# liangxuy/ReGenNet

Hardware: AMD Instinct MI355X
Metric: sampled motions/sec (higher is better)
Workload: dtype bf16 MFMA operands, fp32 accumulate/LayerNorm/softmax, for 990 of 1000 steps; fp16 MFMA operands for the next 8; split-bf16 (x3) for the last 2; 1 GPU; ntu: [B=256/GPU,56,6,60] online/concat/no_cond L8 d512, 1000-step DDPM, Philox noise, hipGraph=on; batch_per_gpu=256, global_batch=256, denoiser_evals_per_motion=1000, parallelism=batch-shard x1

## Files before the change

regennet_amd/csrc/rgn_layers.hip:

```cpp
#include "rgn_internal.h"
#include "rgn_device.h"
#include "rgn_tail.h"
#include "rgn_sampler.h"

#include <hip/hip_runtime.h>

#include <cmath>
#include <type_traits>
#include <utility>

namespace rgn {

#ifndef RGN_LY_ST_AUX
#define RGN_LY_ST_AUX 16
#endif

constexpr int LY_NTH = 512, LY_KB = 4096;
constexpr int LY_X = 0, LY_Y = 64 * 1024, LY_EXCH = LY_Y, LY_RED = 128 * 1024, LY_REDF = 2 * 8 * 64, LY_VEC = LY_RED + 2 * LY_REDF * 4, LY_VECW = 640,
              LY_LDS = 160 * 1024;
constexpr int LY_PF = LY_VEC + 8 * LY_VECW * 4;
static_assert(LY_PF + 8 * 256 <= LY_LDS, "LDS map");
enum { V_BO = 0, V_G1 = 64, V_G2 = 128, V_B2 = 192, V_SPV = 256, V_BF1 = 320 , V_BF2 = 448, V_G3 = 512, V_B3 = 576 };
constexpr int LY_RDA = 6;
constexpr int LY_RDM = 8;
struct LYT {
    static constexpr int MT = 2, NT = 2, NW = 8, R = 64, RD = LY_RDM, KB = LY_KB, RED = LY_RED, REDF = LY_REDF;
};

#ifdef RGN_LY_STAMPS
__device__ long long g_ly_st[1024][16];
#define RGN_LYT(i)                                                                                   \
    {                                                                                                \
        __builtin_amdgcn_sched_barrier(0);                                                           \
        if (threadIdx.x == 0 && blockIdx.x < 1024 && l == RGN_LY_STAMPS) g_ly_st[blockIdx.x][i] = __builtin_readcyclecounter(); \
        __builtin_amdgcn_sched_barrier(0);                                                           \
    }
#define RGN_LYS(i)                                                                                   \
    {                                                                                                \
        __builtin_amdgcn_sched_barrier(0);                                                           \
        if (threadIdx.x == 0 && blockIdx.x < 1024 && it == 1) g_ly_st[blockIdx.x][i] = __builtin_readcyclecounter(); \
        __builtin_amdgcn_sched_barrier(0);                                                           \
    }
#else
#define RGN_LYT(i)
#define RGN_LYS(i)
#endif

constexpr int LY_XLD = 356, LY_TILE = 0, LY_XIMG = 92160, LY_NKX = 11;
static_assert(64 * LY_XLD * 4 <= LY_XIMG && LY_XIMG + LY_NKX * 4096 <= LY_LDS, "step boundary LDS map");

template <bool STEPS, bool GUIDED = false, bool F16 = false, bool INPAINT = false>
__global__ __launch_bounds__(LY_NTH, 2) void k_layers(LayersArgs g) {
    static_assert(STEPS || !GUIDED, "guidance inside the launch needs the step boundary");
    static_assert(STEPS || !INPAINT, "in-painting (rgn_set_inpainting) belongs to the step boundary");
    using OP = OpFmt<F16>;
    using op_t = typename OP::t;
    using op8 = typename OP::v8;
    using op4 = typename OP::v4;
    extern __shared__ __attribute__((aligned(16))) char smem[];
    const int tid = threadIdx.x, lane = tid & 63;
    const int wave = __builtin_amdgcn_readfirstlane(tid >> 6);
    const int wn = wave & 3, hg = wave >> 2;
    const int l31 = lane & 31, kh = lane >> 5;
    const int b = xcd_affine(blockIdx.x, gridDim.x), Tq = g.Tq;
    const size_t row0 = (size_t)b * Tq;
#ifdef RGN_LY_PRIO
    if (wave >= 4) __builtin_amdgcn_s_setprio(RGN_LY_PRIO);
#endif
    float* vec = reinterpret_cast<float*>(smem + LY_VEC) + wave * LY_VECW;
    const int lane16 = lane * 16;
    tile_dma_in(smem + LY_X, g.h, g.rows, row0, Tq, lane, wave);
    const int first_step = (g.stepvec || STEPS) ? *g.d_step : 0;
    const TailLane tl = tail_lane<LYT>(smem, lane, wave);
    static_assert(LY_X == 0, "a_off addresses the image at byte 0");
    int a_off[2], a_offy[2];
    tail_a_off(a_off, lane);
    tail_a_off(a_offy, a_off, LY_Y);
    using Pass = TailPass;
    op8 wf[LY_RDM][2];
    const float qs2 = g.qscale * 1.44269504088896340736f;

    f32x4 qb[4];
    float vb1;
    auto load_qbias = [&](const float* bqkv, int r) {
        const float* bq = bqkv + (2 * r + hg) * 128 + wn * 32;
#pragma unroll
        for (int i4 = 0; i4 < 4; ++i4) qb[i4] = *reinterpret_cast<const f32x4*>(bq + 8 * i4 + 4 * kh);
        vb1 = bq[1024 + l31];
    };

    wait_vmcnt<0>();
    __builtin_amdgcn_s_barrier();
    load_qbias(g.lw[0].bqkv, 0);

    const int nit = STEPS ? g.steps : 1;
    auto out_proj = [&](f32x16 (&acc)[2][2], int wv) {
#pragma unroll
        for (int a2 = 0; a2 < 2; ++a2)
#pragma unroll
            for (int b2 = 0; b2 < 2; ++b2)
#pragma unroll
                for (int i = 0; i < 16; ++i) acc[a2][b2][i] = 0.f;
        if (wv < 6) {
            const int cb0 = 2 * wv;
            const Pass p_out{__builtin_amdgcn_make_buffer_rsrc(const_cast<__bf16*>(g.Wout) + (size_t)cb0 * 1024, 0, (16 * g.nb_out - cb0) * 2048, 0x00020000), LY_NKX * 2048, 0};
#pragma unroll
            for (int s2 = 0; s2 < LY_RDM - 1; ++s2) tail_load_g<OP, LYT>(wf, tl, p_out, s2, s2);
            tail_gemm<OP, LYT, 32, false, 0>(acc, wf, tl, a_off, p_out, p_out);
        }
    };
    for (int it = 0; it < nit; ++it) {
    const int step = first_step - it;
    for (int pass = 0; pass < (GUIDED ? 2 : 1); ++pass) {
    if (GUIDED && pass == 1) {
        f32x16 accp[2][2];
        int wave_p = wave, lane_p = lane, b_p = b;
        asm volatile("" : "+s"(wave_p), "+s"(b_p));
        asm volatile("" : "+v"(lane_p));
        out_proj(accp, wave_p);
        if (wave_p < 6) {
            float* pk = g.park + ((size_t)b_p * 6 + wave_p) * 4096 + lane_p * 4;
#pragma unroll
            for (int nt = 0; nt < 2; ++nt)
#pragma unroll
                for (int mt = 0; mt < 2; ++mt)
#pragma unroll
                    for (int i4 = 0; i4 < 4; ++i4)
                        *reinterpret_cast<f32x4*>(pk + ((nt * 2 + mt) * 4 + i4) * 256) = f32x4{accp[nt][mt][4 * i4], accp[nt][mt][4 * i4 + 1], accp[nt][mt][4 * i4 + 2], accp[nt][mt][4 * i4 + 3]};
        }
        __builtin_amdgcn_s_barrier();
        tile_dma_in<16>(smem + LY_X, g.h, g.rows, g.half + (size_t)b_p * Tq, Tq, lane_p, wave_p);
        wait_vmcnt<0>();
        __builtin_amdgcn_s_barrier();
    }
    for (int l = 0; l < g.L; ++l) {
        const LayerWts& w = g.lw[l];
        RGN_LYT(0)
        op4 attk[2][2][4];
        float bo_r = 0.f;
        {
            struct PassA { __amdgpu_buffer_rsrc_t rs; };
            auto qrs = [&](int r) {
                const int blk = (2 * r + hg) * 4 + wn;
                return __builtin_amdgcn_make_buffer_rsrc(const_cast<__bf16*>(w.Wqkv) + (size_t)blk * 1024, 0, 3 * 512 * 512 * 2 - blk * 2048, 0x00020000);
            };
            const PassA pa[2] = {{qrs(0)}, {qrs(1)}};
            op8 wq[LY_RDA][3];
            auto load_ga = [&](const PassA& ps, int hs, int slot) {
                int soff;
                asm volatile("s_mov_b32 %0, %1" : "=s"(soff) : "i"(frag_granule(hs, 48 * 2048)));
#pragma unroll
                for (int t = 0; t < 3; ++t)
                    wq[slot][t] = __builtin_bit_cast(op8, __builtin_amdgcn_raw_buffer_load_b128(ps.rs, lane16, soff + t * (16 * 2048), 0));
            };
            constexpr int AH = LY_RDA - 1;
#pragma unroll
            for (int s = 0; s < AH; ++s) load_ga(pa[0], s, s);
#pragma unroll
            for (int r = 0; r < 2; ++r) {
                const int head = 2 * r + hg;
                f32x16 acc[2][3];
#pragma unroll
                for (int ta = 0; ta < 2; ++ta)
#pragma unroll
                    for (int i4 = 0; i4 < 4; ++i4)
#pragma unroll
                        for (int e = 0; e < 4; ++e) {
                            acc[ta][0][4 * i4 + e] = qb[i4][e];
                            acc[ta][1][4 * i4 + e] = 0.f;
                            acc[ta][2][4 * i4 + e] = vb1;
                        }
                __builtin_amdgcn_sched_barrier(0);
                {
                    op8 af[2];
#pragma unroll
                    for (int ta = 0; ta < 2; ++ta) af[ta] = *reinterpret_cast<const op8*>(smem + a_off[0] + ta * 2048);
#pragma unroll
                    for (int hs = 0; hs < 32; ++hs) {
                        op8 afn[2];
#pragma unroll
                        for (int ta = 0; ta < 2; ++ta) {
                            afn[ta] = af[ta];
                            if (hs + 1 < 32) afn[ta] = *reinterpret_cast<const op8*>(smem + ((hs + 1) >> 1) * LY_KB + a_off[(hs + 1) & 1] + ta * 2048);
                        }
                        if (hs + AH < 32) load_ga(pa[r], hs + AH, (32 * r + hs + AH) % LY_RDA);
                        else if (r == 0) load_ga(pa[1], hs + AH - 32, (32 * r + hs + AH) % LY_RDA);
                        if (hs + AH < 32 || r == 0) {
                            if (hs < AH) wait_vmcnt<3 * AH + 5>();
                            else wait_vmcnt<3 * AH>();
                        }
                        const int slot = (32 * r + hs) % LY_RDA;
#pragma unroll
                        for (int t = 0; t < 3; ++t)
#pragma unroll
                            for (int ta = 0; ta < 2; ++ta) {
                                if (t < 2) acc[ta][t] = OP::mfma(wq[slot][t], af[ta], acc[ta][t]);
                                else acc[ta][t] = OP::mfma(af[ta], wq[slot][t], acc[ta][t]);
                            }
#pragma unroll
                        for (int ta = 0; ta < 2; ++ta) af[ta] = afn[ta];
                    }
                }
// ... 120 lines not shown
                RGN_LYT(3 + 3 * r)
            }
        }
        const Pass p_wo{tail_wrs(w.Wo, 2 * wave, 512 * 512 * 2), 16 * 2048, 0}, p_w1a{tail_wrs(w.W1, 2 * wave, 1024 * 512 * 2), 32 * 2048, 0},
            p_w1b{tail_wrs(w.W1, 16 + 2 * wave, 1024 * 512 * 2), 32 * 2048, 0}, p_w2a{tail_wrs(w.W2, 2 * wave, 512 * 1024 * 2), 16 * 2048, 0},
            p_w2b{p_w2a.rs, 16 * 2048, 32};
        vec[V_BO + lane] = bo_r;
#pragma unroll
        for (int s = 0; s < LY_RDM - 1; ++s) tail_load_g<OP, LYT>(wf, tl, p_wo, s, s);
        int cw = 64 * wave + lane;
        asm volatile("" : "+v"(cw));
        float vv[12];
        {
            const float* src[9] = {w.bo, w.g1, w.g2, w.b2, w.bf1, w.bf1 + 512, w.bf2, w.g3, w.b3};
            vv[1] = src[1][cw]; vv[2] = src[2][cw]; vv[3] = src[3][cw];
            vv[4] = w.b1[cw] + (g.stepvec ? g.stepvec[(size_t)step * g.ldstep + (size_t)l * 512 + cw] : 0.f) +
                    (g.pervec ? g.pervec[((size_t)b + (size_t)pass * g.B) * g.ldper + (size_t)l * 512 + cw] : 0.f);
            vv[5] = src[4][cw]; vv[6] = src[5][cw]; vv[7] = src[6][cw]; vv[8] = src[7][cw]; vv[9] = src[8][cw];
        }
        asm volatile("" ::: "memory");
#pragma unroll
        for (int r = 0; r < 2; ++r)
#pragma unroll
            for (int qtile = 0; qtile < 2; ++qtile)
#pragma unroll
                for (int i4 = 0; i4 < 4; ++i4)
                    *reinterpret_cast<op4*>(smem + LY_Y + ((2 * r + hg) * 4 + wn) * LY_KB + (32 * qtile + l31) * 64 + img_slot(i4, tl.swz) + 8 * kh) = attk[r][qtile][i4];
        wait_lgkmcnt<0>();
        __builtin_amdgcn_s_barrier();
        f32x16 acc[2][2];
        tail_init_bias<LYT>(acc, tl, vec + V_BO);
        RGN_LYT(7)
        tail_gemm<OP, LYT, 32, true, 11>(acc, wf, tl, a_offy, p_wo, p_w1a);
        RGN_LYT(8)
        vec[V_G1 + lane] = vv[1]; vec[V_G2 + lane] = vv[2]; vec[V_B2 + lane] = vv[3]; vec[V_SPV + lane] = vv[4];
        vec[V_BF1 + lane] = vv[5]; vec[V_BF1 + 64 + lane] = vv[6]; vec[V_BF2 + lane] = vv[7]; vec[V_G3 + lane] = vv[8]; vec[V_B3 + lane] = vv[9];
        tail_add_resid<OP, LYT>(acc, tl, LY_X);
        tail_layernorm<LYT, 0>(acc, tl, vec + V_G1, tail_rowvec(tl, vec + V_SPV));
        tail_layernorm<LYT, 1>(acc, tl, vec + V_G2, tail_rowvec(tl, vec + V_B2));
        tail_store_img<OP, LYT>(acc, tl, LY_X);
        wait_lgkmcnt<0>();
        __builtin_amdgcn_s_barrier();
        RGN_LYT(9)
        f32x16 acc2[2][2];
        tail_ffn<OP, LYT>(acc2, wf, tl, a_off, a_offy, LY_Y, p_w1a, p_w1b, p_w2a, p_w2b, vec + V_BF1, vec + V_BF2);
        load_qbias(g.lw[l + 1 < g.L ? l + 1 : 0].bqkv, 0);
#ifndef RGN_LY_NO_PREFETCH
        if constexpr (STEPS) {
            if (l == g.L - 1) {
                const int nsl = (int)(gridDim.x >> 3) >= 32 ? 32 : ((int)(gridDim.x >> 3) > 0 ? (int)(gridDim.x >> 3) : 1);
                const int sl = (int)(blockIdx.x >> 3) % nsl;
                const int n_out = 16 * g.nb_out * 16, n_all = n_out + LY_NKX * 16 * 16;
                const unsigned pf_lds = (unsigned)(size_t)((RGN_AS3 char*)(smem + LY_PF)) + (unsigned)wave * 256u;
                for (int ln = sl + nsl * tid; ln < n_all; ln += nsl * LY_NTH) {
                    const char* pp = ln < n_out ? reinterpret_cast<const char*>(g.Wout) + (size_t)ln * 128 : reinterpret_cast<const char*>(g.Wx) + (size_t)(ln - n_out) * 128;
                    int m0_keep;
                    asm volatile("s_mov_b32 %0, m0\n\ts_mov_b32 m0, %2\n\ts_nop 0\n\tglobal_load_lds_dword %1, off\n\ts_mov_b32 m0, %0" : "=&s"(m0_keep) : "v"(pp), "s"(pf_lds) : "memory");
                }
            }
        }
#endif
        RGN_LYT(10)
        tail_add_resid<OP, LYT>(acc2, tl, LY_X);
        tail_layernorm<LYT, 0>(acc2, tl, vec + V_G3, tail_rowvec(tl, vec + V_B3));
        tail_store_img<OP, LYT>(acc2, tl, LY_X);
        wait_lgkmcnt<0>();
        __builtin_amdgcn_s_barrier();
        RGN_LYT(11)
    }
    }
    if constexpr (STEPS) {
        int lane_s = lane, wave_s = wave, b_s = b;
        asm volatile("" : "+v"(lane_s));
        asm volatile("" : "+s"(wave_s), "+s"(b_s));
        const int l31_s = lane_s & 31, kh_s = lane_s >> 5;
        const size_t row0_s = (size_t)b_s * Tq;
        auto col4s = [&](int nt, int i4) { return 32 * nt + 8 * i4 + 4 * kh_s; };
        RGN_LYS(12)
        const SampleParams sp = *g.sp;
        const StepCoef k = g.tab[step];
        const int T = Tq, gb = g.s0 + b_s;
        const float gscale = GUIDED ? g.scale[gb] : 0.f;
        const __amdgpu_buffer_rsrc_t park_rs = __builtin_amdgcn_make_buffer_rsrc(GUIDED ? g.park + ((size_t)b_s * 6 + (wave_s < 6 ? wave_s : 0)) * 4096 : nullptr, 0, 4096 * 4, 0x00020000);
        f32x16 acc[2][2];
        out_proj(acc, wave_s);
        __builtin_amdgcn_s_barrier();
        float* tile = reinterpret_cast<float*>(smem + LY_TILE);
#pragma unroll
        for (int nt = 0; nt < 2; ++nt)
#pragma unroll
            for (int i4 = 0; i4 < 4; ++i4) {
                const int n = 64 * wave_s + col4s(nt, i4);
                if (n < 352) {
                    f32x4 bb = {0.f, 0.f, 0.f, 0.f};
                    if (n < g.F) bb = *reinterpret_cast<const f32x4*>(g.bout + n);
#pragma unroll
                    for (int mt = 0; mt < 2; ++mt) {
                        f32x4 v = {acc[nt][mt][4 * i4] + bb[0], acc[nt][mt][4 * i4 + 1] + bb[1], acc[nt][mt][4 * i4 + 2] + bb[2], acc[nt][mt][4 * i4 + 3] + bb[3]};
                        if constexpr (GUIDED) {
                            const f32x4 cc = __builtin_bit_cast(f32x4, __builtin_amdgcn_raw_buffer_load_b128(park_rs, (lane_s * 4 + ((nt * 2 + mt) * 4 + i4) * 256) * 4, 0, 16));
#pragma unroll
                            for (int e = 0; e < 4; ++e) v[e] = guide(cc[e] + bb[e], v[e], gscale);
                        }
                        *reinterpret_cast<f32x4*>(tile + (32 * mt + l31_s) * LY_XLD + n) = v;
                    }
                }
            }
        const Pass p_wx{__builtin_amdgcn_make_buffer_rsrc(const_cast<__bf16*>(g.Wx) + (size_t)(2 * wave_s) * 1024, 0, (LY_NKX * 16 - 2 * wave_s) * 2048, 0x00020000), 16 * 2048, 0};
#pragma unroll
        for (int s2 = 0; s2 < LY_RDM - 1; ++s2) tail_load_g<OP, LYT>(wf, tl, p_wx, s2, s2);
        op4 c0v[2][2][4];
#pragma unroll
        for (int mt = 0; mt < 2; ++mt) {
            const int r = 32 * mt + l31_s, rr = r < T ? r : T - 1;
#pragma unroll
            for (int nt = 0; nt < 2; ++nt)
#pragma unroll
                for (int i4 = 0; i4 < 4; ++i4)
                    c0v[nt][mt][i4] = *reinterpret_cast<const op4*>(g.c0 + (row0_s + rr) * 512 + 64 * wave_s + col4s(nt, i4));
        }
        op4 c0u[GUIDED ? 2 : 1][2][4];
        if constexpr (GUIDED) {
#pragma unroll
            for (int mt = 0; mt < 2; ++mt) {
                const int r = 32 * mt + l31_s, rr = r < T ? r : T - 1;
#pragma unroll
                for (int nt = 0; nt < 2; ++nt)
#pragma unroll
                    for (int i4 = 0; i4 < 4; ++i4)
                        c0u[nt][mt][i4] = *reinterpret_cast<const op4*>(g.c0 + ((size_t)g.half + row0_s + rr) * 512 + 64 * wave_s + col4s(nt, i4));
            }
        }
        wait_lgkmcnt<0>();
        __builtin_amdgcn_s_barrier();
        RGN_LYS(13)
        {
            const int t = lane_s;
            const bool valid = t < T;
            const size_t FT = (size_t)g.F * T;
            const int bn = noise_motion(sp, gb);
            char* ximg = smem + LY_XIMG;
            const int q = lane_s & 3, tq = t - q;
            const bool run4 = valid && (tq & 3) == 0 && tq + 3 < T;
            const bool quads = !sp.noise && !g.no_quads && __all(run4 || tq >= T);
            float xpre[LY_NKX][4];
#pragma unroll
            for (int i2 = 0; i2 < LY_NKX; ++i2)
#pragma unroll
                for (int j = 0; j < 4; ++j) {
                    const int f = 4 * (wave_s + 8 * i2) + j;
                    xpre[i2][j] = (valid && f < g.F) ? sp.x[(size_t)gb * FT + (size_t)f * T + t] : 0.f;
                }
            const int ximg_lane = img_run(lane_s, wave_s >> 1, wave_s & 1);
            constexpr int LY_IPD = GUIDED ? 1 : 2;
            unsigned char mpre[INPAINT ? LY_NKX : 1][4];
            float ipre[INPAINT ? LY_NKX : 1][4];
            const InpaintRsrc irs = inpaint_rsrc(sp, INPAINT ? (size_t)gb * FT : 0, INPAINT ? FT : 0);
            auto inp_request = [&](auto IG) __attribute__((always_inline)) {
                constexpr int ig = decltype(IG)::value;
                if constexpr (INPAINT && ig < LY_NKX) {
#pragma unroll
                    for (int j = 0; j < 4; ++j) inpaint_load(irs, t, (4 * (wave_s + 8 * ig) + j) * T, mpre[ig][j], ipre[ig][j]);
                    asm volatile("" ::: "memory");
                }
            };
            static_for<LY_IPD>([&](auto IG) __attribute__((always_inline)) { inp_request(IG); });
            auto update4 = [&](int i2, int fg, const float (&eps_in)[4], const float (&xv)[4]) {
                op4 nvb;
#pragma unroll
                for (int j = 0; j < 4; ++j) nvb[j] = (op_t)0.f;
                if (valid && 4 * fg < g.F) {
                    const f32x4 x04 = *reinterpret_cast<const f32x4*>(tile + lane_s * LY_XLD + 4 * fg);
#pragma unroll
                    for (int j = 0; j < 4; ++j) {
                        const int f = 4 * fg + j;
                        unsigned char im = 0;
                        float iv = 0.f;
                        if constexpr (INPAINT) { im = mpre[i2][j]; iv = ipre[i2][j]; }
                        const float x0 = pred_x0<INPAINT>(x04[j], im, iv, sp.clip);
                        const size_t o = (size_t)gb * FT + (size_t)f * T + t;
                        if (sp.x0_out) sp.x0_out[o] = x0;
                        const float nv = sampler_next(k, sp.sampler, x0, xv[j], quad_or_step_eps(quads, eps_in[j], sp, step, g.B, FT, bn, f, T, t));
                        sp.x[o] = nv;
                        nvb[j] = (op_t)nv;
                    }
                }
                *reinterpret_cast<op4*>(ximg + i2 * 4096 + ximg_lane) = nvb;
            };
            static_for<LY_NKX>([&](auto IT) __attribute__((always_inline)) {
                constexpr int i2 = decltype(IT)::value;
                const int fg = wave_s + 8 * i2;
                inp_request(std::integral_constant<int, i2 + LY_IPD>{});
                float eps4[4] = {0.f, 0.f, 0.f, 0.f};
                if (quads) quad_normals(sp, step, bn, fg, q, tq, eps4);
                update4(i2, fg, eps4, xpre[i2]);
            });
        }
        wait_lgkmcnt<0>();
        __builtin_amdgcn_s_barrier();
        RGN_LYS(14)
#pragma unroll
        for (int a2 = 0; a2 < 2; ++a2)
#pragma unroll
            for (int b2 = 0; b2 < 2; ++b2)
#pragma unroll
                for (int i = 0; i < 16; ++i) acc[a2][b2][i] = 0.f;
        {
            int a_offx[2] = {a_off[0] + LY_XIMG, a_off[1] + LY_XIMG};
            tail_gemm<OP, LYT, 2 * LY_NKX, false, 8 + 16>(acc, wf, tl, a_offx, p_wx, p_wx);
        }
        if constexpr (GUIDED) {
            __builtin_amdgcn_s_barrier();
#pragma unroll
            for (int nt = 0; nt < 2; ++nt)
#pragma unroll
                for (int i4 = 0; i4 < 4; ++i4)
#pragma unroll
                    for (int mt = 0; mt < 2; ++mt) {
                        op4 hh;
#pragma unroll
                        for (int e = 0; e < 4; ++e) hh[e] = (op_t)(acc[nt][mt][4 * i4 + e] + (float)c0u[nt][mt][i4][e]);
                        *tail_img_run<OP, LYT>(tl, LY_Y, nt, i4, mt) = hh;
                    }
        }
#pragma unroll
        for (int nt = 0; nt < 2; ++nt)
#pragma unroll
            for (int mt = 0; mt < 2; ++mt)
#pragma unroll
                for (int i4 = 0; i4 < 4; ++i4)
#pragma unroll
                    for (int e = 0; e < 4; ++e) acc[nt][mt][4 * i4 + e] += (float)c0v[nt][mt][i4][e];
        tail_store_img<OP, LYT>(acc, tl, LY_X);
        wait_lgkmcnt<0>();
        __builtin_amdgcn_s_barrier();
        if constexpr (GUIDED) {
            const __amdgpu_buffer_rsrc_t u_rs = __builtin_amdgcn_make_buffer_rsrc(g.out, 0, (int)((size_t)g.rows * 512 * 2), 0x00020000);
            const int r16 = lane_s >> 2, c = lane_s & 3;
#pragma unroll
            for (int j = 0; j < 8; ++j) {
                const int p = wave_s * 8 + j, blk = p >> 2, r = (p & 3) * 16 + r16;
                if (r < T) {
                    const int off = blk * LY_KB + r * 64 + ((c ^ ((r >> 2) & 3)) << 4);
                    __builtin_amdgcn_raw_buffer_store_b128(*reinterpret_cast<const u32x4*>(smem + LY_Y + off), u_rs,
                                                           (int)((((size_t)blk * g.rows + g.half + row0_s + r) * 32 + c * 8) * 2), 0, RGN_LY_ST_AUX);
                }
            }
        }
        RGN_LYS(15)
    }
    }
    {
        const __amdgpu_buffer_rsrc_t o_rs = __builtin_amdgcn_make_buffer_rsrc(g.out, 0, (int)((size_t)g.rows * 512 * 2), 0x00020000);
        const int r16 = lane >> 2, c = lane & 3;
#pragma unroll
        for (int j = 0; j < 8; ++j) {
            const int p = wave * 8 + j, blk = p >> 2, r = (p & 3) * 16 + r16;
            if (r < Tq) {
                const int off = blk * LY_KB + img_chunk(r, c);
                __builtin_amdgcn_raw_buffer_store_b128(*reinterpret_cast<const u32x4*>(smem + LY_X + off), o_rs,
                                                       (int)(plane_chunk(g.rows, row0 + r, blk, c) * 2), 0, RGN_LY_ST_AUX);
            }
        }
    }
    if constexpr (STEPS) {
        if (tid == 0) step_ticket(g.d_stepw + 4, (int)gridDim.x, g.d_stepw, first_step - g.steps);
    }
}

#ifdef RGN_LY_STAMPS
void ly_stamps_read(long long* out) { (void)hipMemcpyFromSymbol(out, HIP_SYMBOL(g_ly_st), sizeof(long long) * 1024 * 16); }
#endif

bool layers_supported(int d, int ff, int H, int Tq, int L) { return d == 512 && ff == 1024 && H == 4 && Tq >= 1 && Tq <= 64 && L >= 1 && L <= LY_MAXL; }
bool layers_steps_supported(int d, int F, int Kpx) { return d == 512 && F % 4 == 0 && F <= 352 && Kpx == 32 * LY_NKX; }
constexpr bool layers_form_exists(bool steps, bool guided, bool inpaint) { return steps || !(guided || inpaint); }
template <class Fn>
static hipError_t layers_form(bool steps, bool guided, bool f16, bool inpaint, Fn fn) {
    return dispatch_bools([&](auto S, auto G, auto H, auto I) {
        if constexpr (layers_form_exists(decltype(S)::value, decltype(G)::value, decltype(I)::value))
            return fn(k_layers<decltype(S)::value, decltype(G)::value, decltype(H)::value, decltype(I)::value>);
        else
            return hipErrorInvalidValue;
    }, steps, guided, f16, inpaint);
}
hipError_t configure_layers() {
    hipError_t e = hipSuccess;
    for (int m = 0; m < 16 && e == hipSuccess; ++m)
        if (layers_form_exists(m & 1, m & 2, m & 8))
            e = layers_form(m & 1, m & 2, m & 4, m & 8, [](auto kern) { return hipFuncSetAttribute(reinterpret_cast<const void*>(kern), hipFuncAttributeMaxDynamicSharedMemorySize, LY_LDS); });
    return e;
}
hipError_t launch_layers(const LayersArgs& g, hipStream_t s, bool inpaint) {
    const bool steps = g.steps > 0;
    return layers_form(steps, steps && g.scale, g.f16 != 0, inpaint, [&](auto kern) {
        hipLaunchKernelGGL(kern, dim3(g.Bm), dim3(LY_NTH), LY_LDS, s, g);
        return hipGetLastError();
    });
}

}
```

regennet_amd/csrc/rgn_layout.h:

```cpp
#pragma once
#include <cstddef>

#if defined(__HIP__) || defined(__CUDACC__)
#define RGN_HD __attribute__((host)) __attribute__((device))
#else
#define RGN_HD
#endif

namespace rgn {

template <class T> struct layout_index { typedef T type; };

template <class I = size_t>
RGN_HD constexpr inline I plane_chunk(typename layout_index<I>::type rows, typename layout_index<I>::type row, int kb, int chunk) {
    return ((I)kb * rows + row) * 32 + chunk * 8;
}
template <class I = size_t>
RGN_HD constexpr inline I plane_off(typename layout_index<I>::type rows, typename layout_index<I>::type row, int col) {
    return ((I)(col >> 5) * rows + row) * 32 + (col & 31);
}

RGN_HD constexpr inline int img_swz(int row) { return (row >> 2) & 3; }
RGN_HD constexpr inline int img_slot(int chunk, int swz) { return (chunk ^ swz) << 4; }
RGN_HD constexpr inline int img_chunk(int row, int chunk) { return row * 64 + img_slot(chunk, img_swz(row)); }
RGN_HD constexpr inline int img_frag(int row, int ks, int kh) { return row * 64 + img_slot(2 * ks + kh, img_swz(row)); }
RGN_HD constexpr inline int img_run(int row, int i4, int kh) { return row * 64 + img_slot(i4, img_swz(row)) + 8 * kh; }
RGN_HD constexpr inline int img_dma_chunk(int row, int slot) { return slot ^ img_swz(row); }

RGN_HD constexpr inline int frag_lane(int n, int k) { return 32 * ((k % 16) / 8) + n % 32; }
RGN_HD constexpr inline int frag_elem(int k) { return k % 8; }
RGN_HD constexpr inline size_t frag_off(size_t nb_all, int n, int k) {
    return ((((size_t)(k / 32) * nb_all + n / 32) * 2 + (k % 32) / 16) * 64 + frag_lane(n, k)) * 8 + frag_elem(k);
}
RGN_HD constexpr inline int frag_granule(int hs, int kstride) { return (hs >> 1) * kstride + (hs & 1) * 1024; }

RGN_HD constexpr inline int mfma32_row(int i, int kh) { return (i & 3) + 8 * (i >> 2) + 4 * kh; }
RGN_HD constexpr inline int mfma32_col(int lane) { return lane & 31; }

namespace layout_detail {
constexpr bool chunks_permute() {
    for (int r = 0; r < 64; ++r) {
        int seen = 0;
        for (int c = 0; c < 4; ++c) {
            seen |= 1 << ((img_chunk(r, c) - r * 64) >> 4);
            if (img_chunk(r, img_dma_chunk(r, c)) != r * 64 + c * 16) return false;
        }
        if (seen != 15) return false;
    }
    return true;
}
constexpr bool roles_agree() {
    for (int r = 0; r < 64; ++r)
        for (int ks = 0; ks < 2; ++ks)
            for (int kh = 0; kh < 2; ++kh) {
                if (img_frag(r, ks, kh) != img_chunk(r, 2 * ks + kh)) return false;
                if (img_run(r, 2 * ks + kh, 1) != img_chunk(r, 2 * ks + kh) + 8) return false;
            }
    return true;
}
constexpr bool cd_rows_permute() {
    unsigned seen = 0;
    for (int i = 0; i < 16; ++i)
        for (int kh = 0; kh < 2; ++kh) seen |= 1u << mfma32_row(i, kh);
    return seen == 0xffffffffu;
}
}
static_assert(layout_detail::chunks_permute(), "the chunk map permutes 0 .. 3 in every row and the DMA source rule inverts it");
static_assert(layout_detail::roles_agree(), "fragment (r, ks, kh) is logical chunk 2 ks + kh; an accumulator run is half a chunk");
static_assert(layout_detail::cd_rows_permute(), "the C/D row map covers the 32 rows of a tile");
static_assert(plane_off(300, 7, 37) == plane_chunk(300, 7, 1, 0) + 5, "a plane element lies in chunk (col % 32) / 8 of k-block col / 32");
static_assert(frag_off(16, 33, 49) * 2 == frag_granule(3, 16 * 2048) + 2048 + frag_lane(33, 49) * 16 + frag_elem(49) * 2, "granule, column block, lane, element");

}
```

regennet_amd/csrc/rgn_tail.h:

```cpp
#pragma once
#include "rgn_device.h"

namespace rgn {
namespace {

struct TailLane {
    char* smem;
    int lane16, wave, kh, swz;
    int img_base;
    int red_base;
    int red_base2;
};
template <class C>
__device__ __forceinline__ TailLane tail_lane(char* smem, int lane, int wave) {
    const int l31 = lane & 31, kh = lane >> 5;
    int img_base = (C::NT * wave) * C::KB + l31 * 64 + 8 * kh;
    asm volatile("" : "+v"(img_base));
    int red_base = C::RED + 4 * l31;
    asm volatile("" : "+v"(red_base));
    int red_base2 = red_base + 128 * kh;
    asm volatile("" : "+v"(red_base2));
    return TailLane{smem, lane * 16, wave, kh, img_swz(l31), img_base, red_base, red_base2};
}

__device__ __forceinline__ void tail_a_off(int (&a)[2], int lane) {
    const int l31 = lane & 31, kh = lane >> 5;
#pragma unroll
    for (int ks = 0; ks < 2; ++ks) a[ks] = img_frag(l31, ks, kh);
}
__device__ __forceinline__ void tail_a_off(int (&a)[2], const int (&a0)[2], int img) {
#pragma unroll
    for (int ks = 0; ks < 2; ++ks) a[ks] = a0[ks] + img;
}
__device__ __forceinline__ int tail_col4(const TailLane& t, int nt, int i4) { return 32 * nt + 8 * i4 + 4 * t.kh; }
template <class OP, class C>
__device__ __forceinline__ typename OP::v4* tail_img_run(const TailLane& t, int img, int nt, int i4, int mt) {
    return reinterpret_cast<typename OP::v4*>(t.smem + (img + t.img_base + img_slot(i4, t.swz)) + (nt * C::KB + mt * 2048));
}

struct TailPass { __amdgpu_buffer_rsrc_t rs; int kstride, hs0; };
__device__ __forceinline__ __amdgpu_buffer_rsrc_t tail_wrs(const __bf16* W, int cb0, int bytes) {
    return __builtin_amdgcn_make_buffer_rsrc(const_cast<__bf16*>(W) + (size_t)cb0 * 1024, 0, bytes - cb0 * 2048, 0x00020000);
}
template <class OP, class C>
__device__ __forceinline__ void tail_load_g(typename OP::v8 (&wf)[C::RD][C::NT], const TailLane& t, const TailPass& ps, int hs_rel, int slot) {
    const int hs = ps.hs0 + hs_rel;
    int soff;
    asm volatile("s_mov_b32 %0, %1" : "=s"(soff) : "i"(frag_granule(hs, ps.kstride)));
#pragma unroll
    for (int nt = 0; nt < C::NT; ++nt)
        wf[slot][nt] = __builtin_bit_cast(typename OP::v8, __builtin_amdgcn_raw_buffer_load_b128(ps.rs, t.lane16, soff + nt * 2048, 0));
}
template <class OP, class C, int NG, bool CH, int EX>
__device__ __forceinline__ void tail_gemm(f32x16 (&acc)[C::NT][C::MT], typename OP::v8 (&wf)[C::RD][C::NT], const TailLane& t, const int (&aoff)[2],
                                          const TailPass& cur, const TailPass& nxt) {
    using op8 = typename OP::v8;
    constexpr int MT = C::MT, NT = C::NT, RD = C::RD, AH = RD - 1;
    __builtin_amdgcn_sched_barrier(0);
    op8 af[MT];
#pragma unroll
    for (int mt = 0; mt < MT; ++mt) af[mt] = *reinterpret_cast<const op8*>(t.smem + aoff[0] + mt * 2048);
#pragma unroll
    for (int hs = 0; hs < NG; ++hs) {
        op8 afn[MT];
#pragma unroll
        for (int mt = 0; mt < MT; ++mt) {
            afn[mt] = af[mt];
            if (hs + 1 < NG) afn[mt] = *reinterpret_cast<const op8*>(t.smem + ((hs + 1) >> 1) * C::KB + aoff[(hs + 1) & 1] + mt * 2048);
        }
        if (hs + AH < NG) tail_load_g<OP, C>(wf, t, cur, hs + AH, (hs + AH) % RD);
        else if (CH) tail_load_g<OP, C>(wf, t, nxt, hs + AH - NG, (hs + AH) % RD);
        if (hs + AH < NG || CH) {
            if (hs < AH) wait_vmcnt<NT * AH + EX>();
            else wait_vmcnt<NT * AH>();
        }
#pragma unroll
        for (int nt = 0; nt < NT; ++nt)
#pragma unroll
            for (int mt = 0; mt < MT; ++mt) acc[nt][mt] = OP::mfma(wf[hs % RD][nt], af[mt], acc[nt][mt]);
#pragma unroll
        for (int mt = 0; mt < MT; ++mt) af[mt] = afn[mt];
    }
    __builtin_amdgcn_sched_barrier(0);
}

template <class C>
__device__ __forceinline__ void tail_init_bias(f32x16 (&acc)[C::NT][C::MT], const TailLane& t, const float* bias) {
#pragma unroll
    for (int nt = 0; nt < C::NT; ++nt)
#pragma unroll
        for (int i4 = 0; i4 < 4; ++i4) {
            const f32x4 b = *reinterpret_cast<const f32x4*>(bias + tail_col4(t, nt, i4));
#pragma unroll
            for (int mt = 0; mt < C::MT; ++mt)
#pragma unroll
                for (int e = 0; e < 4; ++e) acc[nt][mt][4 * i4 + e] = b[e];
        }
}
template <class C, int SLOT, class Shift>
__device__ __forceinline__ void tail_layernorm(f32x16 (&acc)[C::NT][C::MT], const TailLane& t, const float* gam, Shift shift) {
    constexpr int MT = C::MT, NT = C::NT, NW = C::NW, R = C::R;
    static_assert(MT == 2, "the two half_swaps hand over exactly two row tiles");
    const char* buf = t.smem + t.red_base + SLOT * C::REDF * 4;
    const char* buf2 = t.smem + t.red_base2 + SLOT * C::REDF * 4;
    const float invn = 1.0f / 512.f;
#pragma unroll
    for (int mt = 0; mt < MT; ++mt) {
        f32x2 s2 = f32x2{0.f, 0.f}, q2 = f32x2{0.f, 0.f};
#pragma unroll
        for (int nt = 0; nt < NT; ++nt)
#pragma unroll
            for (int i = 0; i < 16; i += 2) {
                const f32x2 v = f32x2{acc[nt][mt][i], acc[nt][mt][i + 1]};
                s2 += v;
                q2 = __builtin_elementwise_fma(v, v, q2);
            }
        float s = s2[0] + s2[1], q = q2[0] + q2[1];
        half_swap(s, q);
        *reinterpret_cast<float*>(const_cast<char*>(buf) + (t.kh * (NW * R) + t.wave * R + 32 * mt) * 4) = s + q;
    }
    wait_lgkmcnt<0>();
    __builtin_amdgcn_s_barrier();
    f32x2 rs[MT], nm[MT];
    {
        float p[2][NW];
#pragma unroll
        for (int st = 0; st < 2; ++st)
#pragma unroll
            for (int w = 0; w < NW; ++w) p[st][w] = *reinterpret_cast<const float*>(buf2 + (st * (NW * R) + w * R) * 4);
#pragma unroll
        for (int st = 0; st < 2; ++st)
#pragma unroll
            for (int d = 1; d < NW; d *= 2)
#pragma unroll
                for (int w = 0; w < NW; w += 2 * d) p[st][w] += p[st][w + d];
        const float mean = p[0][0] * invn;
        const float var = __builtin_fmaxf(p[1][0] * invn - mean * mean, 0.f);
        float r0 = __builtin_amdgcn_rsqf(var + 1e-5f), n0 = -mean * r0;
        float r1 = r0, n1 = n0;
        asm volatile("" : "+v"(r1), "+v"(n1));
        half_swap(r0, r1);
        half_swap(n0, n1);
        rs[0] = f32x2{r0, r0}; rs[1] = f32x2{r1, r1};
        nm[0] = f32x2{n0, n0}; nm[1] = f32x2{n1, n1};
    }
#pragma unroll
    for (int nt = 0; nt < NT; ++nt) {
        f32x4 ga[4], sh[4][MT];
#pragma unroll
        for (int i4 = 0; i4 < 4; ++i4) {
            ga[i4] = *reinterpret_cast<const f32x4*>(gam + tail_col4(t, nt, i4));
#pragma unroll
            for (int mt = 0; mt < MT; ++mt) sh[i4][mt] = shift(nt, i4, mt);
        }
// ... 86 lines not shown
```

Measured before the change: 502.3 motions/s.

## Overlap Philox noise draws with output projection and fuse sampler update into GEMM epilogue

Generates the per-step Gaussian noise (Philox plus Box-Muller) in rounds spread across waves and interleaves it into the output-projection GEMM loop through a new hook, staging the noise in an LDS buffer. The sampler update now runs directly from the MFMA accumulator registers instead of going through an fp32 LDS tile and a second pass. x, guidance and inpaint loads are prefetched with buffer loads, and the new sample is written straight into the A-image used by the Wx GEMM. The goal is to hide the noise ALU work under the GEMM's memory waits and to remove a barrier-separated LDS round trip at each step boundary. The cost is higher register pressure and a new LDS layout that could hurt occupancy or scheduling.

```diff
diff --git a/regennet_amd/csrc/rgn_layers.hip b/regennet_amd/csrc/rgn_layers.hip
--- a/regennet_amd/csrc/rgn_layers.hip
+++ b/regennet_amd/csrc/rgn_layers.hip
@@ -29,6 +29,7 @@
 
 #ifdef RGN_LY_STAMPS
 __device__ long long g_ly_st[1024][16];
+__device__ int g_ly_it = 1;
 #define RGN_LYT(i)                                                                                   \
     {                                                                                                \
         __builtin_amdgcn_sched_barrier(0);                                                           \
@@ -38,7 +39,7 @@
 #define RGN_LYS(i)                                                                                   \
     {                                                                                                \
         __builtin_amdgcn_sched_barrier(0);                                                           \
-        if (threadIdx.x == 0 && blockIdx.x < 1024 && it == 1) g_ly_st[blockIdx.x][i] = __builtin_readcyclecounter(); \
+        if (threadIdx.x == 0 && blockIdx.x < 1024 && it == g_ly_it) g_ly_st[blockIdx.x][i] = __builtin_readcyclecounter(); \
         __builtin_amdgcn_sched_barrier(0);                                                           \
     }
 #else
@@ -46,8 +47,8 @@
 #define RGN_LYS(i)
 #endif
 
-constexpr int LY_XLD = 356, LY_TILE = 0, LY_XIMG = 92160, LY_NKX = 11;
-static_assert(64 * LY_XLD * 4 <= LY_XIMG && LY_XIMG + LY_NKX * 4096 <= LY_LDS, "step boundary LDS map");
+constexpr int LY_E = LY_Y, LY_BOUT = LY_E + BU_E_BYTES, LY_NKX = 11;
+static_assert(LY_BOUT + BU_FMAX * 4 <= LY_PF && LY_NKX * LY_KB <= LY_Y && 32 * LY_NKX == BU_FMAX, "step boundary LDS map");
 
 template <bool STEPS, bool GUIDED = false, bool F16 = false, bool INPAINT = false>
 __global__ __launch_bounds__(LY_NTH, 2) void k_layers(LayersArgs g) {
@@ -94,7 +95,7 @@
     load_qbias(g.lw[0].bqkv, 0);
 
     const int nit = STEPS ? g.steps : 1;
-    auto out_proj = [&](f32x16 (&acc)[2][2], int wv) {
+    auto out_proj = [&](f32x16 (&acc)[2][2], int wv, auto hook) {
 #pragma unroll
         for (int a2 = 0; a2 < 2; ++a2)
 #pragma unroll
@@ -106,7 +107,7 @@
             const Pass p_out{__builtin_amdgcn_make_buffer_rsrc(const_cast<__bf16*>(g.Wout) + (size_t)cb0 * 1024, 0, (16 * g.nb_out - cb0) * 2048, 0x00020000), LY_NKX * 2048, 0};
 #pragma unroll
             for (int s2 = 0; s2 < LY_RDM - 1; ++s2) tail_load_g<OP, LYT>(wf, tl, p_out, s2, s2);
-            tail_gemm<OP, LYT, 32, false, 0>(acc, wf, tl, a_off, p_out, p_out);
+            tail_gemm<OP, LYT, 32, false, 0>(acc, wf, tl, a_off, p_out, p_out, hook);
         }
     };
     for (int it = 0; it < nit; ++it) {
@@ -117,7 +118,7 @@
         int wave_p = wave, lane_p = lane, b_p = b;
         asm volatile("" : "+s"(wave_p), "+s"(b_p));
         asm volatile("" : "+v"(lane_p));
-        out_proj(accp, wave_p);
+        out_proj(accp, wave_p, TailNoHook{});
         if (wave_p < 6) {
             float* pk = g.park + ((size_t)b_p * 6 + wave_p) * 4096 + lane_p * 4;
 #pragma unroll
@@ -404,37 +405,169 @@
         const int T = Tq, gb = g.s0 + b_s;
         const float gscale = GUIDED ? g.scale[gb] : 0.f;
         const __amdgpu_buffer_rsrc_t park_rs = __builtin_amdgcn_make_buffer_rsrc(GUIDED ? g.park + ((size_t)b_s * 6 + (wave_s < 6 ? wave_s : 0)) * 4096 : nullptr, 0, 4096 * 4, 0x00020000);
+        const size_t FT = (size_t)g.F * T;
+        const int bn = noise_motion(sp, gb);
+        const bool draws = !sp.noise && !g.no_quads;
+        const int tid_s = 64 * wave_s + lane_s;
+        const float bout_s = tid_s < g.F ? g.bout[tid_s] : 0.f;
         f32x16 acc[2][2];
-        out_proj(acc, wave_s);
-        __builtin_amdgcn_s_barrier();
-        float* tile = reinterpret_cast<float*>(smem + LY_TILE);
-#pragma unroll
-        for (int nt = 0; nt < 2; ++nt)
-#pragma unroll
-            for (int i4 = 0; i4 < 4; ++i4) {
-                const int n = 64 * wave_s + col4s(nt, i4);
-                if (n < 352) {
-                    f32x4 bb = {0.f, 0.f, 0.f, 0.f};
-                    if (n < g.F) bb = *reinterpret_cast<const f32x4*>(g.bout + n);
+        {
+            const int nj = bu_quads(T), nun = g.F * nj, rounds = draws ? bu_rounds(g.F, T) : 0;
+            const int rd0 = bu_first_round(rounds, wave_s), rd1 = bu_first_round(rounds, wave_s + 1), nrw = rd1 - rd0;
+            int rd = rd0;
+            const unsigned magic = bu_magic(nj);
+            const unsigned long long sample = sp.sample_offset + bn;
+            auto draw_round = [&]() __attribute__((always_inline)) {
+                const int u = rd * 64 + lane_s;
+                ++rd;
+                if (u < nun) {
+                    const int f = bu_unit_f(u, magic), j = u - f * nj;
+                    uint32_t r[4];
+                    philox4x32_10(noise_elem(f, 4 * j) >> 2, (uint32_t)step, (uint32_t)sample, (uint32_t)(sample >> 32), (uint32_t)sp.seed, (uint32_t)(sp.seed >> 32), r);
+                    float n0, n1, n2, n3;
+                    box_muller(r[0], r[1], n0, n1);
+                    box_muller(r[2], r[3], n2, n3);
+                    *reinterpret_cast<f32x4*>(smem + LY_E + bu_e_off(f, 4 * j)) = f32x4{n0, n1, n2, n3};
+                }
+            };
+            auto hook = [&](int hs) __attribute__((always_inline)) {
+                while (rd < rd1 && (rd - rd0) * 32 < (hs + 1) * nrw) draw_round();
+            };
+            out_proj(acc, wave_s, hook);
+            while (rd < rd1) draw_round();
+        }
+        if (tid_s < BU_FMAX) *reinterpret_cast<float*>(smem + LY_BOUT + tid_s * 4) = bout_s;
+        const int fw = 64 * wave_s + 4 * kh_s, eT = 4 * T;
+        const __amdgpu_buffer_rsrc_t x_rs = __builtin_amdgcn_make_buffer_rsrc(sp.x + (size_t)gb * FT, 0, wave_s < 6 ? (int)(FT * 4) : 0, 0x00020000);
+        const __amdgpu_buffer_rsrc_t x0_rs = __builtin_amdgcn_make_buffer_rsrc(sp.x0_out + (size_t)gb * FT, 0, sp.x0_out ? (int)(FT * 4) : 0, 0x00020000);
+        const InpaintRsrc irs = inpaint_rsrc(sp, INPAINT ? (size_t)gb * FT : 0, INPAINT ? FT : 0);
+        bool rowv[2];
+        int tcl[2];
+#pragma unroll
+        for (int mt = 0; mt < 2; ++mt) {
+            const int r = 32 * mt + l31_s;
+            rowv[mt] = r < T;
+            tcl[mt] = r < T ? r : T - 1;
+        }
+        auto elem = [&](int gi, int mt) {
+            const int f4 = fw + 8 * gi;
+            return (f4 < g.F ? f4 : g.F - 4) * T + tcl[mt];
+        };
+        float xv[8][2][4];
+        f32x4 cc[GUIDED ? 8 : 1][2];
+        constexpr int LY_IPD = 1, LY_CPD = 1, LY_XPD = INPAINT ? (GUIDED ? 2 : 4) : 8;
+        unsigned char mpre[INPAINT ? 8 : 1][2][4];
+        float ipre[INPAINT ? 8 : 1][2][4];
+        auto inp_request = [&](auto GI) __attribute__((always_inline)) {
+            constexpr int gi = decltype(GI)::value;
+            if constexpr (INPAINT && gi < 8) {
+#pragma unroll
+                for (int mt = 0; mt < 2; ++mt) {
+                    const int el = elem(gi, mt);
+#pragma unroll
+                    for (int e = 0; e < 4; ++e) inpaint_load(irs, el, e * T, mpre[gi][mt][e], ipre[gi][mt][e]);
+                }
+                asm volatile("" ::: "memory");
+            }
+        };
+        const Pass p_wx{__builtin_amdgcn_make_buffer_rsrc(const_cast<__bf16*>(g.Wx) + (size_t)(2 * wave_s) * 1024, 0, (LY_NKX * 16 - 2 * wave_s) * 2048, 0x00020000), 16 * 2048, 0};
+        auto x_request = [&](auto GI) __attribute__((always_inline)) {
+            constexpr int gi = decltype(GI)::value;
+            if constexpr (gi < 8) {
+#pragma unroll
+                for (int mt = 0; mt < 2; ++mt) {
+                    const int el = elem(gi, mt);
+#pragma unroll
+                    for (int e = 0; e < 4; ++e) xv[gi][mt][e] = __builtin_bit_cast(float, __builtin_amdgcn_raw_buffer_load_b32(x_rs, el * 4, e * eT, 0));
+                }
+                asm volatile("" ::: "memory");
+            }
+        };
+        auto c_request = [&](auto GI) __attribute__((always_inline)) {
+            constexpr int gi = decltype(GI)::value;
+            if constexpr (GUIDED && gi < 8) {
+#pragma unroll
+                for (int mt = 0; mt < 2; ++mt)
+                    cc[gi][mt] = __builtin_bit_cast(f32x4, __builtin_amdgcn_raw_buffer_load_b128(park_rs, (lane_s * 4 + (((gi >> 2) * 2 + mt) * 4 + (gi & 3)) * 256) * 4, 0, 16));
+                asm volatile("" ::: "memory");
+            }
+        };
+        static_for<LY_XPD>([&](auto GI) __attribute__((always_inline)) { x_request(GI); });
+        static_for<LY_CPD>([&](auto GI) __attribute__((always_inline)) { c_request(GI); });
+        static_for<LY_IPD>([&](auto GI) __attribute__((always_inline)) { inp_request(GI); });
+        wait_lgkmcnt<0>();
+        __builtin_amdgcn_s_barrier();
+        RGN_LYS(13)
+        if (wave_s < 6) {
+            if (!draws) {
+#pragma unroll 1
+                for (int gi = 0; gi < 8; ++gi) {
+                    const int n = fw + 8 * gi;
 #pragma unroll
                     for (int mt = 0; mt < 2; ++mt) {
-                        f32x4 v = {acc[nt][mt][4 * i4] + bb[0], acc[nt][mt][4 * i4 + 1] + bb[1], acc[nt][mt][4 * i4 + 2] + bb[2], acc[nt][mt][4 * i4 + 3] + bb[3]};
-                        if constexpr (GUIDED) {
-                            const f32x4 cc = __builtin_bit_cast(f32x4, __builtin_amdgcn_raw_buffer_load_b128(park_rs, (lane_s * 4 + ((nt * 2 + mt) * 4 + i4) * 256) * 4, 0, 16));
-#pragma unroll
-                            for (int e = 0; e < 4; ++e) v[e] = guide(cc[e] + bb[e], v[e], gscale);
-                        }
-                        *reinterpret_cast<f32x4*>(tile + (32 * mt + l31_s) * LY_XLD + n) = v;
-                    }
-                }
-            }
-        const Pass p_wx{__builtin_amdgcn_make_buffer_rsrc(const_cast<__bf16*>(g.Wx) + (size_t)(2 * wave_s) * 1024, 0, (LY_NKX * 16 - 2 * wave_s) * 2048, 0x00020000), 16 * 2048, 0};
+                        const int t = 32 * mt + l31_s;
+                        if (rowv[mt] && n < g.F) {
+#pragma unroll
+                            for (int e = 0; e < 4; ++e) *reinterpret_cast<float*>(smem + LY_E + bu_e_off(n + e, t)) = step_eps(sp, step, g.B, FT, bn, n + e, T, t);
+                        }
+                    }
+                }
+                wait_vmcnt<0>();
+                wait_lgkmcnt<0>();
+            }
+            static_for<8>([&](auto GI) __attribute__((always_inline)) {
+                constexpr int gi = decltype(GI)::value, nt = gi >> 2, i4 = gi & 3;
+                x_request(std::integral_constant<int, gi + LY_XPD>{});
+                c_request(std::integral_constant<int, gi + LY_CPD>{});
+                inp_request(std::integral_constant<int, gi + LY_IPD>{});
+                const int n = fw + 8 * gi;
+                const f32x4 bb = *reinterpret_cast<const f32x4*>(smem + LY_BOUT + n * 4);
+                const bool fv = n < g.F;
+#pragma unroll
+                for (int mt = 0; mt < 2; ++mt) {
+                    const int t = 32 * mt + l31_s;
+                    float ev[4];
+#pragma unroll
+                    for (int e = 0; e < 4; ++e) ev[e] = *reinterpret_cast<const float*>(smem + LY_E + bu_e_off(n + e, t));
+                    f32x4 v = {acc[nt][mt][4 * i4] + bb[0], acc[nt][mt][4 * i4 + 1] + bb[1], acc[nt][mt][4 * i4 + 2] + bb[2], acc[nt][mt][4 * i4 + 3] + bb[3]};
+                    if constexpr (GUIDED) {
+#pragma unroll
+                        for (int e = 0; e < 4; ++e) v[e] = guide(cc[gi][mt][e] + bb[e], v[e], gscale);
+                    }
+                    op4 nvb;
+#pragma unroll
+                    for (int e = 0; e < 4; ++e) nvb[e] = (op_t)0.f;
+                    if (rowv[mt] && fv) {
+                        const int el4 = (n * T + t) * 4;
+                        float x0[4];
+#pragma unroll
+                        for (int e = 0; e < 4; ++e) {
+                            unsigned char im = 0;
+                            float iv = 0.f;
+                            if constexpr (INPAINT) { im = mpre[gi][mt][e]; iv = ipre[gi][mt][e]; }
+                            x0[e] = pred_x0<INPAINT>(v[e], im, iv, sp.clip);
+                        }
+                        if (sp.x0_out) {
+#pragma unroll
+                            for (int e = 0; e < 4; ++e) __builtin_amdgcn_raw_buffer_store_b32(__builtin_bit_cast(int, x0[e]), x0_rs, el4, e * eT, 0);
+                        }
+#pragma unroll
+                        for (int e = 0; e < 4; ++e) {
+                            const float nv = sampler_next(k, sp.sampler, x0[e], xv[gi][mt][e], ev[e]);
+                            __builtin_amdgcn_raw_buffer_store_b32(__builtin_bit_cast(int, nv), x_rs, el4, e * eT, 0);
+                            nvb[e] = (op_t)nv;
+                        }
+                    }
+                    if (2 * wave_s + nt < LY_NKX) *tail_img_run<OP, LYT>(tl, LY_X, nt, i4, mt) = nvb;
+                }
+            });
+        }
 #pragma unroll
         for (int s2 = 0; s2 < LY_RDM - 1; ++s2) tail_load_g<OP, LYT>(wf, tl, p_wx, s2, s2);
         op4 c0v[2][2][4];
 #pragma unroll
         for (int mt = 0; mt < 2; ++mt) {
-            const int r = 32 * mt + l31_s, rr = r < T ? r : T - 1;
+            const int rr = tcl[mt];
 #pragma unroll
             for (int nt = 0; nt < 2; ++nt)
 #pragma unroll
@@ -445,7 +578,7 @@
         if constexpr (GUIDED) {
 #pragma unroll
             for (int mt = 0; mt < 2; ++mt) {
-                const int r = 32 * mt + l31_s, rr = r < T ? r : T - 1;
+                const int rr = tcl[mt];
 #pragma unroll
                 for (int nt = 0; nt < 2; ++nt)
 #pragma unroll
@@ -455,71 +588,6 @@
         }
         wait_lgkmcnt<0>();
         __builtin_amdgcn_s_barrier();
-        RGN_LYS(13)
-        {
-            const int t = lane_s;
-            const bool valid = t < T;
-            const size_t FT = (size_t)g.F * T;
-            const int bn = noise_motion(sp, gb);
-            char* ximg = smem + LY_XIMG;
-            const int q = lane_s & 3, tq = t - q;
-            const bool run4 = valid && (tq & 3) == 0 && tq + 3 < T;
-            const bool quads = !sp.noise && !g.no_quads && __all(run4 || tq >= T);
-            float xpre[LY_NKX][4];
-#pragma unroll
-            for (int i2 = 0; i2 < LY_NKX; ++i2)
-#pragma unroll
-                for (int j = 0; j < 4; ++j) {
-                    const int f = 4 * (wave_s + 8 * i2) + j;
-                    xpre[i2][j] = (valid && f < g.F) ? sp.x[(size_t)gb * FT + (size_t)f * T + t] : 0.f;
-                }
-            const int ximg_lane = img_run(lane_s, wave_s >> 1, wave_s & 1);
-            constexpr int LY_IPD = GUIDED ? 1 : 2;
-            unsigned char mpre[INPAINT ? LY_NKX : 1][4];
-            float ipre[INPAINT ? LY_NKX : 1][4];
-            const InpaintRsrc irs = inpaint_rsrc(sp, INPAINT ? (size_t)gb * FT : 0, INPAINT ? FT : 0);
-            auto inp_request = [&](auto IG) __attribute__((always_inline)) {
-                constexpr int ig = decltype(IG)::value;
-                if constexpr (INPAINT && ig < LY_NKX) {
-#pragma unroll
-                    for (int j = 0; j < 4; ++j) inpaint_load(irs, t, (4 * (wave_s + 8 * ig) + j) * T, mpre[ig][j], ipre[ig][j]);
-                    asm volatile("" ::: "memory");
-                }
-            };
-            static_for<LY_IPD>([&](auto IG) __attribute__((always_inline)) { inp_request(IG); });
-            auto update4 = [&](int i2, int fg, const float (&eps_in)[4], const float (&xv)[4]) {
-                op4 nvb;
-#pragma unroll
-                for (int j = 0; j < 4; ++j) nvb[j] = (op_t)0.f;
-                if (valid && 4 * fg < g.F) {
-                    const f32x4 x04 = *reinterpret_cast<const f32x4*>(tile + lane_s * LY_XLD + 4 * fg);
-#pragma unroll
-                    for (int j = 0; j < 4; ++j) {
-                        const int f = 4 * fg + j;
-                        unsigned char im = 0;
-                        float iv = 0.f;
-                        if constexpr (INPAINT) { im = mpre[i2][j]; iv = ipre[i2][j]; }
-                        const float x0 = pred_x0<INPAINT>(x04[j], im, iv, sp.clip);
-                        const size_t o = (size_t)gb * FT + (size_t)f * T + t;
-                        if (sp.x0_out) sp.x0_out[o] = x0;
-                        const float nv = sampler_next(k, sp.sampler, x0, xv[j], quad_or_step_eps(quads, eps_in[j], sp, step, g.B, FT, bn, f, T, t));
-                        sp.x[o] = nv;
-                        nvb[j] = (op_t)nv;
-                    }
-                }
-                *reinterpret_cast<op4*>(ximg + i2 * 4096 + ximg_lane) = nvb;
-            };
-            static_for<LY_NKX>([&](auto IT) __attribute__((always_inline)) {
-                constexpr int i2 = decltype(IT)::value;
-                const int fg = wave_s + 8 * i2;
-                inp_request(std::integral_constant<int, i2 + LY_IPD>{});
-                float eps4[4] = {0.f, 0.f, 0.f, 0.f};
-                if (quads) quad_normals(sp, step, bn, fg, q, tq, eps4);
-                update4(i2, fg, eps4, xpre[i2]);
-            });
-        }
-        wait_lgkmcnt<0>();
-        __builtin_amdgcn_s_barrier();
         RGN_LYS(14)
 #pragma unroll
         for (int a2 = 0; a2 < 2; ++a2)
@@ -527,12 +595,9 @@
             for (int b2 = 0; b2 < 2; ++b2)
 #pragma unroll
                 for (int i = 0; i < 16; ++i) acc[a2][b2][i] = 0.f;
-        {
-            int a_offx[2] = {a_off[0] + LY_XIMG, a_off[1] + LY_XIMG};
-            tail_gemm<OP, LYT, 2 * LY_NKX, false, 8 + 16>(acc, wf, tl, a_offx, p_wx, p_wx);
-        }
+        tail_gemm<OP, LYT, 2 * LY_NKX, false, 16>(acc, wf, tl, a_off, p_wx, p_wx);
+        __builtin_amdgcn_s_barrier();
         if constexpr (GUIDED) {
-            __builtin_amdgcn_s_barrier();
 #pragma unroll
             for (int nt = 0; nt < 2; ++nt)
 #pragma unroll
@@ -591,6 +656,7 @@
 }
 
 #ifdef RGN_LY_STAMPS
+void ly_stamps_iter(int it) { (void)hipMemcpyToSymbol(HIP_SYMBOL(g_ly_it), &it, sizeof(int)); }
 void ly_stamps_read(long long* out) { (void)hipMemcpyFromSymbol(out, HIP_SYMBOL(g_ly_st), sizeof(long long) * 1024 * 16); }
 #endif
 
diff --git a/regennet_amd/csrc/rgn_layout.h b/regennet_amd/csrc/rgn_layout.h
--- a/regennet_amd/csrc/rgn_layout.h
+++ b/regennet_amd/csrc/rgn_layout.h
@@ -37,6 +37,20 @@
 RGN_HD constexpr inline int mfma32_row(int i, int kh) { return (i & 3) + 8 * (i >> 2) + 4 * kh; }
 RGN_HD constexpr inline int mfma32_col(int lane) { return lane & 31; }
 
+constexpr int BU_LD = 64, BU_FMAX = 352, BU_E_BYTES = BU_FMAX * BU_LD * 4, BU_S23 = 2;
+RGN_HD constexpr inline int bu_quads(int T) { return (T + 3) >> 2; }
+RGN_HD constexpr inline int bu_rounds(int F, int T) { return (F * bu_quads(T) + 63) >> 6; }
+RGN_HD constexpr inline int bu_share(int wave) { return (wave & 2) ? ((wave & 4) ? 8 - BU_S23 : BU_S23) : 4; }
+RGN_HD constexpr inline int bu_share_before(int wave) {
+    int c = 0;
+    for (int i = 0; i < 8; ++i) c += i < wave ? bu_share(i) : 0;
+    return c;
+}
+RGN_HD constexpr inline int bu_first_round(int rounds, int wave) { return rounds * bu_share_before(wave) >> 5; }
+RGN_HD constexpr inline unsigned bu_magic(int nj) { return (262144u + (unsigned)nj - 1u) / (unsigned)nj; }
+RGN_HD constexpr inline int bu_unit_f(int u, unsigned magic) { return (int)(((unsigned)u * magic) >> 18); }
+RGN_HD constexpr inline int bu_e_off(int f, int t) { return (f * BU_LD + t) * 4; }
+
 namespace layout_detail {
 constexpr bool chunks_permute() {
     for (int r = 0; r < 64; ++r) {
@@ -68,6 +82,8 @@
 static_assert(layout_detail::chunks_permute(), "the chunk map permutes 0 .. 3 in every row and the DMA source rule inverts it");
 static_assert(layout_detail::roles_agree(), "fragment (r, ks, kh) is logical chunk 2 ks + kh; an accumulator run is half a chunk");
 static_assert(layout_detail::cd_rows_permute(), "the C/D row map covers the 32 rows of a tile");
+static_assert(bu_share_before(8) == 32 && bu_share(0) + bu_share(4) == 8 && bu_share(2) + bu_share(6) == 8 && bu_first_round(79, 8) == 79, "every SIMD draws a quarter of the rounds");
+static_assert(bu_unit_f(5631, bu_magic(16)) == 351 && bu_unit_f(5039, bu_magic(15)) == 335 && bu_e_off(BU_FMAX - 1, BU_LD - 4) + 16 == BU_E_BYTES, "unit split and the end of E");
 static_assert(plane_off(300, 7, 37) == plane_chunk(300, 7, 1, 0) + 5, "a plane element lies in chunk (col % 32) / 8 of k-block col / 32");
 static_assert(frag_off(16, 33, 49) * 2 == frag_granule(3, 16 * 2048) + 2048 + frag_lane(33, 49) * 16 + frag_elem(49) * 2, "granule, column block, lane, element");
 
diff --git a/regennet_amd/csrc/rgn_tail.h b/regennet_amd/csrc/rgn_tail.h
--- a/regennet_amd/csrc/rgn_tail.h
+++ b/regennet_amd/csrc/rgn_tail.h
@@ -1,5 +1,7 @@
 #pragma once
 #include "rgn_device.h"
+
+#include <type_traits>
 
 namespace rgn {
 namespace {
@@ -51,9 +53,10 @@
     for (int nt = 0; nt < C::NT; ++nt)
         wf[slot][nt] = __builtin_bit_cast(typename OP::v8, __builtin_amdgcn_raw_buffer_load_b128(ps.rs, t.lane16, soff + nt * 2048, 0));
 }
-template <class OP, class C, int NG, bool CH, int EX>
+struct TailNoHook {};
+template <class OP, class C, int NG, bool CH, int EX, class Hook = TailNoHook>
 __device__ __forceinline__ void tail_gemm(f32x16 (&acc)[C::NT][C::MT], typename OP::v8 (&wf)[C::RD][C::NT], const TailLane& t, const int (&aoff)[2],
-                                          const TailPass& cur, const TailPass& nxt) {
+                                          const TailPass& cur, const TailPass& nxt, Hook hook = Hook{}) {
     using op8 = typename OP::v8;
     constexpr int MT = C::MT, NT = C::NT, RD = C::RD, AH = RD - 1;
     __builtin_amdgcn_sched_barrier(0);
@@ -70,6 +73,7 @@
         }
         if (hs + AH < NG) tail_load_g<OP, C>(wf, t, cur, hs + AH, (hs + AH) % RD);
         else if (CH) tail_load_g<OP, C>(wf, t, nxt, hs + AH - NG, (hs + AH) % RD);
+        if constexpr (!std::is_same_v<Hook, TailNoHook>) hook(hs);
         if (hs + AH < NG || CH) {
             if (hs < AH) wait_vmcnt<NT * AH + EX>();
             else wait_vmcnt<NT * AH>();
```

Result: no change. 506.8 motions/s, median of 6 (+0.9%).
